# amcolex/ofdm-sync-math

Measured on AMD Instinct MI355X. Metric: complex Msamples/s through S&C metric kernel @ batch=65536; % HBM roofline, higher is better.
Workload: dtype f32 (c64 in, f64 prefix sums); 1 GPU; cfg3 Schmidl-Cox float32 metric+CFO, N=1024 (L=512), cir1, 65536 streams x 1024 c64 per GPU; global_batch=65536, seq_len=1024, L=512, parallelism=stream-shard x1 (no collectives), placement=auto -> contiguous

## Files before the change

### ofdm-sync-math_amd/csrc/aa_fast.hip

```cpp
#include "ofs_common.h"
#include "aa_gate.h"
#include "ofdmsync.h"

using namespace ofs;

namespace {

#ifndef OFS_FAST_WG
#define OFS_FAST_WG 64
#endif
constexpr int FAST_WG = OFS_FAST_WG;

#ifndef OFS_FAST_WAVES
#define OFS_FAST_WAVES 0
#endif
#if OFS_FAST_WAVES > 0
#define OFS_FAST_BOUNDS __launch_bounds__(FAST_WG, OFS_FAST_WAVES)
#else
#define OFS_FAST_BOUNDS __launch_bounds__(FAST_WG)
#endif
constexpr int TMAX = 1024;
constexpr int FAST_CAP_LDS = 160 * 1024 / 10;

#ifndef OFS_DMA_AUX
#define OFS_DMA_AUX 0
#endif
#ifndef OFS_FAST_STAGE
#define OFS_FAST_STAGE 1
#endif
typedef float nf4 __attribute__((ext_vector_type(4)));
typedef float nf2 __attribute__((ext_vector_type(2)));
typedef float pf2 __attribute__((ext_vector_type(2)));
__device__ __forceinline__ pf2 mulc_acc(pf2 c, pf2 d, pf2 acc) {
    acc = __builtin_elementwise_fma(c, d.xx, acc);
    return __builtin_elementwise_fma(c.yx, pf2{d.y, -d.y}, acc);
}
template <int SP>
__device__ __forceinline__ void st_out(float4* p, float4 v) {
    const nf4 d = nf4{v.x, v.y, v.z, v.w};
    if constexpr (SP == 1) __builtin_nontemporal_store(d, reinterpret_cast<nf4*>(p));
    else *p = v;
}
template <int SP>
__device__ __forceinline__ void st_out(float2* p, float2 v) {
    const nf2 d = nf2{v.x, v.y};
    if constexpr (SP == 1) __builtin_nontemporal_store(d, reinterpret_cast<nf2*>(p));
    else *p = v;
}

template <int SP>
__device__ __forceinline__ void st_rows2(float* span, const float (&a)[2], const float (&b)[2], int lane) {
    const bool odd = (lane & 1) != 0;
    const int idx = (lane < 32 ? 2 * lane : 2 * lane - 63) * 4;
    float o[4];
#pragma unroll
    for (int e = 0; e < 2; ++e) {
        const int ai = __float_as_int(a[e]), bi = __float_as_int(b[e]);
        const int bdn = dpp_i<0xA0>(bi);
        const int aup = dpp_i<0xF5>(ai);
        const int we = odd ? bdn : ai;
        const int wo = odd ? bi : aup;
        o[e] = __int_as_float(__builtin_amdgcn_ds_bpermute(idx, we));
        o[2 + e] = __int_as_float(__builtin_amdgcn_ds_bpermute(idx, wo));
    }
    st_out<SP>(reinterpret_cast<float4*>(span) + lane, make_float4(o[0], o[1], o[2], o[3]));
}


#ifndef OFS_FAST_FF
#define OFS_FAST_FF 0
#endif
#ifndef OFS_FAST_GATE_LATE
#define OFS_FAST_GATE_LATE 0
#endif
#ifndef OFS_FAST_HEADSCAN
#define OFS_FAST_HEADSCAN 0
#endif
template <int E, int MR, int NA, bool DO, bool S32, int SV = 0>
__global__ OFS_FAST_BOUNDS void aa_fast_kernel(AaFastArgs a) {
    static_assert(SV == 0 || (E == 2 && NA == 1 && !DO), "store-path variants: one-antenna E = 2 storing kernel");
    constexpr int SP = SV & 1;
    constexpr bool RP = (SV & 2) != 0;
    constexpr int RL = 64 * E;
    constexpr int RW = TMAX / RL;
    constexpr int L = MR * RL;
    constexpr int V4 = E / 2;
    static_assert(MR >= 1 && MR <= RW, "window must fit the stream tile");
#if OFS_FAST_STAGE == 0
    __shared__ float4 lds[FAST_WG / 64][NA * RW * V4][64];
#endif
    const int lane = threadIdx.x & 63;
    const int w = threadIdx.x >> 6;
    const int64_t b = (int64_t)(NA == 1 ? blockIdx.x : xcd_block()) * (FAST_WG / 64) + w;
    if (b >= a.B) return;
    const int T = (int)a.T;
#if OFS_FAST_STAGE == 0
    constexpr int SPR = V4 + ((E % 4 != 0) ? 2 * V4 : 2 * (V4 / 2));
#pragma unroll
    for (int k = 0; k < RW; ++k)
#pragma unroll
        for (int t = 0; t < NA; ++t) {
            const float2* xs = reinterpret_cast<const float2*>(a.x) + (b * NA + t) * a.T;
#pragma unroll
            for (int j = 0; j < V4; ++j) {
                int n = RL * k + E * lane + 2 * j;
                n = n < T ? n : T - 2;
                ofs::lds_dma16(xs + n, &lds[w][(t * RW + k) * V4 + j][0]);
            }
        }
    auto ldrow = [&](int t, int k, int j) { return lds[w][(t * RW + k) * V4 + j][lane]; };
    const bool all_out = !DO && !RP && a.P && a.R && a.M;
    auto row_wait = [&](int k) {
        if (all_out) ofs::vmcnt_wait((RW - 1 - k) * NA * V4 + k * SPR);
        else ofs::vmcnt_wait((RW - 1 - k) * NA * V4);
    };
#elif OFS_FAST_STAGE == 2
    constexpr int SPR = V4 + ((E % 4 != 0) ? 2 * V4 : 2 * (V4 / 2));
    nf4 xreg[NA][RW][V4];
#pragma unroll
    for (int k = 0; k < RW; ++k)
#pragma unroll
        for (int t = 0; t < NA; ++t) {
            const float2* xs = reinterpret_cast<const float2*>(a.x) + (b * NA + t) * a.T;
#pragma unroll
            for (int j = 0; j < V4; ++j) {
                int n = RL * k + E * lane + 2 * j;
                n = n < T ? n : T - 2;
                asm volatile("global_load_dwordx4 %0, %1, off" : "=v"(xreg[t][k][j]) : "v"(xs + n) : "memory");
            }
        }
    const bool count_st = !DO && !RP && a.P && a.R && a.M && T == TMAX;
    auto ldrow = [&](int t, int k, int j) { const nf4 v = xreg[t][k][j]; return make_float4(v.x, v.y, v.z, v.w); };
    auto row_wait = [&](int k) {
        if (count_st) ofs::vmcnt_wait((RW - 1 - k) * NA * V4 + k * SPR);
        else ofs::vmcnt_wait((RW - 1 - k) * NA * V4);
#pragma unroll
        for (int t = 0; t < NA; ++t)
#pragma unroll
            for (int j = 0; j < V4; ++j) asm volatile("" : "+v"(xreg[t][k][j]));
    };
#else
    float4 xreg[NA][RW][V4];
#pragma unroll
    for (int t = 0; t < NA; ++t) {
        const float2* xs = reinterpret_cast<const float2*>(a.x) + (b * NA + t) * a.T;
#pragma unroll
        for (int k = 0; k < RW; ++k)
#pragma unroll
            for (int j = 0; j < V4; ++j) {
                int n = RL * k + E * lane + 2 * j;
                n = n < T ? n : T - 2;
                xreg[t][k][j] = *reinterpret_cast<const float4*>(xs + n);
            }
    }
    auto ldrow = [&](int t, int k, int j) { return xreg[t][k][j]; };
    auto row_wait = [&](int) {};
#endif
    auto xrow = [&](int t, int k, pf2 (&c)[E]) {
#pragma unroll
        for (int j = 0; j < V4; ++j) {
            const bool ok = RL * k + E * lane + 2 * j < T;
            const float4 v = ldrow(t, k, j);
            c[2 * j] = ok ? pf2{v.x, v.y} : pf2{0.f, 0.f};
            c[2 * j + 1] = ok ? pf2{v.z, v.w} : pf2{0.f, 0.f};
        }
    };

    pf2 sS[MR][E];
    float sE[MR][E];
    double Cr[RW + 1], Ci[RW + 1], Ce[RW + 1];
    Cr[0] = Ci[0] = Ce[0] = 0.0;

    AaRowGate<E, float, false, (bool)(DO || OFS_FAST_FF || NA == 1)> gate;
#if OFS_FAST_GATE_LATE
    constexpr int GR = RW - MR > 0 ? RW - MR : 1;
    __shared__ float4 gl[FAST_WG / 64][GR][E][64];
#endif
    if (a.detect)
        gate.init(a.hyst, L, a.thr, a.fs, a.max_ev, a.ev_i + b * (int64_t)a.max_ev * 4,
                  a.ev_r + b * (int64_t)a.max_ev * 4);

    float* Pout = DO ? nullptr : reinterpret_cast<float*>(a.P);
    float* Rout = DO ? nullptr : reinterpret_cast<float*>(a.R);
    float* Mout = DO ? nullptr : reinterpret_cast<float*>(a.M);
    const float floor_ = 1e-6f * (float)L;
    float hR[2] = {0.f, 0.f}, hM[2] = {0.f, 0.f};
    const bool head = !DO && a.head_resident != 0;

#pragma unroll
    for (int k = 0; k < RW; ++k) {
        if (RL * k < T) {
            const int nb = RL * k + E * lane;
            pf2 av[E];
            float aE[E];
#pragma unroll
            for (int e = 0; e < E; ++e) { av[e] = pf2{0.f, 0.f}; aE[e] = 0.f; }
            row_wait(k);
#pragma unroll
            for (int t = 0; t < NA; ++t) {
                pf2 c[E];
                xrow(t, k, c);
#pragma unroll
                for (int e = 0; e < E; ++e) aE[e] += fmaf(c[e].x, c[e].x, c[e].y * c[e].y);
                if (k >= MR) {
                    pf2 d[E];
                    xrow(t, k - MR, d);
#pragma unroll
                    for (int e = 0; e < E; ++e) av[e] = mulc_acc(c[e], d[e], av[e]);
                }
            }
            pf2 fS[E], gS[E];
            float fE[E], gE[E];
            fS[0] = av[0]; fE[0] = aE[0];
#pragma unroll
            for (int e = 1; e < E; ++e) { fS[e] = fS[e - 1] + av[e]; fE[e] = fE[e - 1] + aE[e]; }
            gS[E - 1] = pf2{0.f, 0.f}; gE[E - 1] = 0.f;
#pragma unroll
            for (int e = E - 2; e >= 0; --e) { gS[e] = gS[e + 1] + av[e + 1]; gE[e] = gE[e + 1] + aE[e + 1]; }
            const RowScan sEr = row_scan<S32>(fE[E - 1]);
            RowScan sRr{0.f, 0.f, 0.0}, sIr{0.f, 0.f, 0.0};
            if (k >= MR || OFS_FAST_HEADSCAN) { sRr = row_scan<S32>(fS[E - 1].x); sIr = row_scan<S32>(fS[E - 1].y); }
            const double totR = sRr.tot, totI = sIr.tot, totE = sEr.tot;
            const pf2 xS = pf2{sRr.x, sIr.x};
            const float xE = sEr.x;
            const pf2 uS = pf2{sRr.u, sIr.u};
            const float uE = sEr.u;
            Cr[k + 1] = Cr[k] + totR; Ci[k + 1] = Ci[k] + totI; Ce[k + 1] = Ce[k] + totE;
            const pf2 wS = pf2{(float)((k >= MR) ? (Cr[k] - Cr[k - MR + 1]) : Cr[k]),
                               (float)((k >= MR) ? (Ci[k] - Ci[k - MR + 1]) : Ci[k])};
            const float wE = (float)((k >= MR) ? (Ce[k] - Ce[k - MR + 1]) : Ce[k]);

            float pf[E][2], mf[E], pmf[E], rf[E];
#pragma unroll
            for (int e = 0; e < E; ++e) {
                pf2 P = wS + (xS + fS[e]);
                float RR = wE + (xE + fE[e]);
                if (k >= MR) { P += sS[k % MR][e]; RR += sE[k % MR][e]; }
                sS[k % MR][e] = uS + gS[e]; sE[k % MR][e] = uE + gE[e];
                const float pm = fmaf(P.x, P.x, P.y * P.y);
                float m = 0.f;
                if (k >= MR && RR > floor_) m = fminf(pm * __builtin_amdgcn_rcpf(RR * RR), 1.f);
                pf[e][0] = P.x; pf[e][1] = P.y; rf[e] = RR; mf[e] = m; pmf[e] = pm;
            }

            const int64_t o = b * a.T + nb;
            float* const Pk = (k < MR && head) ? nullptr : Pout;
            float* const Mk = (k < MR && head) ? nullptr : Mout;
            const bool paired = RP && (T & 3) == 0 && RL * ((k & ~1) + 2) <= T;
#pragma unroll
            for (int j = 0; j < V4; ++j) {
                if (nb + 2 * j < T) {
                    if (Pk) st_out<SP>(reinterpret_cast<float4*>(Pk + 2 * (o + 2 * j)),
                                         make_float4(pf[2 * j][0], pf[2 * j][1], pf[2 * j + 1][0], pf[2 * j + 1][1]));
                    if (paired) {
                    } else if (E % 4 != 0 || (T & 3) != 0) {
                        if (Rout) st_out<SP>(reinterpret_cast<float2*>(Rout + o + 2 * j), make_float2(rf[2 * j], rf[2 * j + 1]));
                        if (Mk) st_out<SP>(reinterpret_cast<float2*>(Mk + o + 2 * j), make_float2(mf[2 * j], mf[2 * j + 1]));
                    } else if ((j & 1) == 0) {
                        if (Rout) st_out<SP>(reinterpret_cast<float4*>(Rout + o + 2 * j),
                                             make_float4(rf[2 * j], rf[2 * j + 1], rf[2 * j + 2], rf[2 * j + 3]));
                        if (Mk) st_out<SP>(reinterpret_cast<float4*>(Mk + o + 2 * j),
                                             make_float4(mf[2 * j], mf[2 * j + 1], mf[2 * j + 2], mf[2 * j + 3]));
                    }
                    if (!DO && a.valid) { a.valid[o + 2 * j] = (k >= MR); a.valid[o + 2 * j + 1] = (k >= MR); }
                }
            }
            if constexpr (RP) {
                if (paired) {
                    if ((k & 1) == 0) {
                        hR[0] = rf[0]; hR[1] = rf[1]; hM[0] = mf[0]; hM[1] = mf[1];
                    } else {
                        const int64_t o0 = b * a.T + RL * (k - 1);
                        if (Rout) st_rows2<SP>(Rout + o0, hR, rf, lane);
                        if (Mk) st_rows2<SP>(Mk + o0, hM, mf, lane);
                    }
                }
            }

            if (a.detect && k >= MR) {
#if OFS_FAST_GATE_LATE
#pragma unroll
                for (int e = 0; e < E; ++e) gl[w][k >= MR ? k - MR : 0][e][lane] = make_float4(mf[e], pmf[e], pf[e][0], pf[e][1]);
#else
                float pr[E], pi[E];
#pragma unroll
                for (int e = 0; e < E; ++e) { pr[e] = pf[e][0]; pi[e] = pf[e][1]; }
                gate.row(lane, k, nb, T, mf, pmf, pr, pi);
#endif
            }
        }
    }
#if OFS_FAST_GATE_LATE
    if (a.detect) {
        __builtin_amdgcn_fence(__ATOMIC_RELEASE, "wavefront");
        __builtin_amdgcn_wave_barrier();
        __builtin_amdgcn_fence(__ATOMIC_ACQUIRE, "wavefront");
#pragma unroll 1
        for (int k = MR; k < RW; ++k) {
            if (RL * k >= T) break;
            float m[E], pm[E], pr[E], pi[E];
#pragma unroll
            for (int e = 0; e < E; ++e) {
                const float4 v = gl[w][k - MR][e][lane];
                m[e] = v.x; pm[e] = v.y; pr[e] = v.z; pi[e] = v.w;
            }
            gate.row(lane, k, RL * k + E * lane, T, m, pm, pr, pi);
        }
    }
#endif
    if (a.detect) gate.finish(lane, T, a.n_ev + b);
}

typedef float f4u __attribute__((ext_vector_type(4), aligned(8)));
typedef float f2u __attribute__((ext_vector_type(2), aligned(4)));

#ifndef OFS_STREAM_WG
#define OFS_STREAM_WG 64
#endif
constexpr int STREAM_WG = OFS_STREAM_WG;
#ifndef OFS_STREAM_PD
#define OFS_STREAM_PD 0
#endif
#ifndef OFS_STREAM_WAVES
#define OFS_STREAM_WAVES 0
#endif
#ifndef OFS_STREAM_WG1
#define OFS_STREAM_WG1 128
#endif
constexpr int stream_wg(int na, bool det_only) { return (na == 1 && !det_only) ? OFS_STREAM_WG1 : STREAM_WG; }
#if OFS_STREAM_WAVES > 0
#define OFS_STREAM_BOUNDS __launch_bounds__(stream_wg(NA, DO), OFS_STREAM_WAVES)
#else
#define OFS_STREAM_BOUNDS __launch_bounds__(stream_wg(NA, DO))
#endif

#ifndef OFS_STREAM_FF
#define OFS_STREAM_FF 1
#endif
#ifndef OFS_STREAM_LDSLAG
#define OFS_STREAM_LDSLAG 1
#endif

template <int E, int MR, int NA, bool DO>
struct AaStream {
    static constexpr int RL = 64 * E;
    static constexpr int L = MR * RL;
    static constexpr int V4 = E / 2;
    static constexpr int PD = OFS_STREAM_PD > 0 ? OFS_STREAM_PD : ((E == 2 && NA == 2) ? 4 : 2);
    static constexpr int PER = MR > PD ? MR : PD;
    static constexpr bool LDSLAG = OFS_STREAM_LDSLAG == 2 || (OFS_STREAM_LDSLAG == 1 && NA == 2);

    const float2* xb;
    float4 (*lag)[NA][V4][64];
    int64_t T, o0;
    int Ti, nrows, full_rows, lane;
    pf2 lx[LDSLAG ? 1 : NA][MR][E];
    pf2 sS[MR][E];
    float sE[MR][E];
    double cbR[MR], cbI[MR], cbE[MR];
    double CR, CI, CE;
    float2 nx[PD][NA][E];
    AaRowGate<E, float, false, (bool)(DO || OFS_STREAM_FF)> gate;
    float2* Pout; float* Rout; float* Mout; uint8_t* Vout;
// ... 170 lines not shown
        if (p < s.nrows) s.load_row(p, s.nx[p]);
    s.detect = a.detect != 0;
    if (s.detect)
        s.gate.init(a.hyst, S::L, a.thr, a.fs, a.max_ev, a.ev_i + b * (int64_t)a.max_ev * 4,
                    a.ev_r + b * (int64_t)a.max_ev * 4);
    s.Pout = DO ? nullptr : reinterpret_cast<float2*>(a.P);
    s.Rout = DO ? nullptr : reinterpret_cast<float*>(a.R);
    s.Mout = DO ? nullptr : reinterpret_cast<float*>(a.M);
    s.Vout = DO ? nullptr : a.valid;
    s.head = !DO && a.head_resident != 0;
    s.floor_ = 1e-6f * (float)S::L;

    s.template block<true, true>(0);
    int k0 = S::PER;
    for (; k0 + S::PER + S::PD <= s.full_rows; k0 += S::PER) s.template block<false, false>(k0);
    for (; k0 < s.nrows; k0 += S::PER) s.template block<false, true>(k0);
    if (a.detect) s.gate.finish(lane, s.Ti, a.n_ev + b);
}

template <int E, int MR, int NA>
int launch_stream(const AaFastArgs& a, hipStream_t st) {
    const bool det_only = a.detect && !a.P && !a.R && !a.M && !a.valid;
    constexpr int WGD = stream_wg(NA, true), WGS = stream_wg(NA, false);
    const int64_t grid = det_only ? (a.B + WGD / 64 - 1) / (WGD / 64) : (a.B + WGS / 64 - 1) / (WGS / 64);
    using S = AaStream<E, MR, NA, false>;
    constexpr size_t lag_lds = (size_t)(WGS / 64) * (S::LDSLAG ? MR : 1) * NA * S::V4 * 64 * 16;
    constexpr size_t cap_total = 24 * 1024;
    const size_t dflt = (!det_only && NA == 2 && cap_total > lag_lds) ? cap_total - lag_lds : 0;
    const size_t shm = ofs::variant(ofs::V_OCC_LDS) == INT64_MIN ? dflt : ofs::occ_lds();
    if (det_only)
        hipLaunchKernelGGL((aa_stream_kernel<E, MR, NA, true>), dim3((unsigned)grid), dim3(WGD), shm, st, a);
    else
        hipLaunchKernelGGL((aa_stream_kernel<E, MR, NA, false>), dim3((unsigned)grid), dim3(WGS), shm, st, a);
    return hipGetLastError() == hipSuccess ? 1 : OFS_EHIP;
}

template <int E, int NA>
int launch_stream_mr(int mr, const AaFastArgs& a, hipStream_t st) {
    switch (mr) {
        case 1: return launch_stream<E, 1, NA>(a, st);
        case 2: return launch_stream<E, 2, NA>(a, st);
        case 4: return launch_stream<E, 4, NA>(a, st);
        case 8: return launch_stream<E, 8, NA>(a, st);
    }
    return 0;
}

bool scan32(bool det_only) {
    const int64_t v = ofs::variant(det_only ? ofs::V_FAST_SCAN_DO : ofs::V_FAST_SCAN);
    if (v == 32 || v == 64) return v == 32;
    return det_only;
}

template <int E, int MR, int NA>
int launch(const AaFastArgs& a, hipStream_t st) {
    const bool det_only = a.detect && !a.P && !a.R && !a.M && !a.valid;
    const bool s32 = scan32(det_only);
    const dim3 grid((unsigned)((a.B + FAST_WG / 64 - 1) / (FAST_WG / 64))), blk(FAST_WG);
    const int64_t pad = ofs::variant_or(ofs::V_FAST_LDS, (!det_only && NA == 1) ? FAST_CAP_LDS : 0);
    const size_t shm = pad > 0 && pad <= 65536 ? (size_t)pad : 0;
    if constexpr (E == 2 && NA == 1) {
        if (!det_only && !s32) {
            const int sv = (ofs::variant_or(ofs::V_FAST_RMPAIR, 1) != 0 ? 2 : 0) | (ofs::variant_or(ofs::V_FAST_ST_POLICY, 1) == 1 ? 1 : 0);
            switch (sv) {
                case 0: hipLaunchKernelGGL((aa_fast_kernel<E, MR, NA, false, false, 0>), grid, blk, shm, st, a); break;
                case 1: hipLaunchKernelGGL((aa_fast_kernel<E, MR, NA, false, false, 1>), grid, blk, shm, st, a); break;
                case 2: hipLaunchKernelGGL((aa_fast_kernel<E, MR, NA, false, false, 2>), grid, blk, shm, st, a); break;
                default: hipLaunchKernelGGL((aa_fast_kernel<E, MR, NA, false, false, 3>), grid, blk, shm, st, a);
            }
            return hipGetLastError() == hipSuccess ? 1 : OFS_EHIP;
        }
    }
    if (det_only && s32) hipLaunchKernelGGL((aa_fast_kernel<E, MR, NA, true, true>), grid, blk, shm, st, a);
    else if (det_only) hipLaunchKernelGGL((aa_fast_kernel<E, MR, NA, true, false>), grid, blk, shm, st, a);
    else if (s32) hipLaunchKernelGGL((aa_fast_kernel<E, MR, NA, false, true>), grid, blk, shm, st, a);
    else hipLaunchKernelGGL((aa_fast_kernel<E, MR, NA, false, false>), grid, blk, shm, st, a);
    return hipGetLastError() == hipSuccess ? 1 : OFS_EHIP;
}

template <int E, int NA, int MR = 1>
int launch_mr(int mr, const AaFastArgs& a, hipStream_t st) {
    if constexpr (MR > TMAX / (64 * E)) {
        return 0;
    } else {
        if (mr == MR) return launch<E, MR, NA>(a, st);
        return launch_mr<E, NA, MR + 1>(mr, a, st);
    }
}

template <int NA>
int launch_e(int E, int mr, const AaFastArgs& a, hipStream_t st) {
    switch (E) {
        case 2: return launch_mr<2, NA>(mr, a, st);
        case 4: return launch_mr<4, NA>(mr, a, st);
        case 8: return launch_mr<8, NA>(mr, a, st);
    }
    return 0;
}

int pick_e(int L) {
    const int forced = (int)ofs::variant_or(ofs::V_FAST_E, 0);
    if (forced == 2 || forced == 4 || forced == 8) return (L % (64 * forced) == 0) ? forced : 0;
    for (int e : {2, 4, 8})
        if (L % (64 * e) == 0) return e;
    return 0;
}

int pick_e_do(int L) {
    const int forced = (int)ofs::variant_or(ofs::V_FAST_E_DO, 0);
    for (int e : {forced, 4, 8, 2})
        if ((e == 2 || e == 4 || e == 8) && L % (64 * e) == 0) return e;
    return 0;
}

}

// ... 33 lines not shown
```

### ofdm-sync-math_amd/csrc/aa_gate.h

```cpp
#pragma once
#include "ofs_common.h"

namespace ofs {

#ifndef OFS_GATE_FASTFLAGS
#define OFS_GATE_FASTFLAGS 1
#endif
#ifndef OFS_GATE_PRED
#define OFS_GATE_PRED 0
#endif
#ifndef OFS_GATE_NOINLINE_EMIT
#define OFS_GATE_NOINLINE_EMIT 0
#endif
#ifndef OFS_GATE_FFONLY
#define OFS_GATE_FFONLY 0
#endif
#ifndef OFS_GATE_DIAG
#define OFS_GATE_DIAG 0
#endif
#ifndef OFS_GATE_NOACC
#define OFS_GATE_NOACC 0
#endif
#ifndef OFS_GATE_DEFER
#define OFS_GATE_DEFER 1
// ... 25 lines not shown
        lane_reset();
    }

#if OFS_GATE_NOINLINE_EMIT
    __device__ __attribute__((noinline)) void emit(int lane, int gate_end) {
#else
    __device__ __forceinline__ void emit(int lane, int gate_end) {
#endif
        if (evi && n_ev < max_ev && lane < 8) {
            int64_t* ei = evi + (int64_t)n_ev * 4;
            if constexpr (RTL) {
                const int64_t f[4] = {bidx, (int64_t)bidx + toff, ev_start, (int64_t)gate_end + 1};
                if (lane < 4) ei[lane] = f[lane & 3];
            } else {
                double* er = evr + (int64_t)n_ev * 4;
                const int64_t f[4] = {out_peak(), out_start(), out_pos(gate_end), out_peak() - 2 * L + 1};
                if (lane < 4) {
                    ei[lane] = f[lane & 3];
                } else {
                    const double ang = sizeof(V) == 4 ? (double)fast_atan2f((float)bpi, (float)bpr)
                                                      : atan2((double)bpi, (double)bpr);
                    const double g[4] = {(double)bpr, (double)bpi, (double)bm, ang * fs / (2.0 * M_PI * (double)L)};
                    er[lane - 4] = g[lane & 3];
                }
            }
        }
        n_ev += 1;
    }

    __device__ __forceinline__ void row(int lane, int k, int nb, int T, const V (&m)[E], const V (&pm)[E],
                                        const V (&pr)[E], const V (&pi)[E]) {
#if OFS_GATE_DIAG == 1
        return;
#endif
        bool ab[E];
#pragma unroll
        for (int e = 0; e < E; ++e) ab[e] = (nb + e < T) && (double)m[e] >= thr;
#if OFS_GATE_DIAG == 2
        uint64_t any = 0;
#pragma unroll
        for (int e = 0; e < E; ++e) any |= __ballot(ab[e]);
        if (any) carry_last = RL * k;
        return;
#endif
        row_flags(lane, k, nb, T, ab, pm, pr, pi, m);
    }

    V lv, lpr, lpi, lm;
    int lk;
    __device__ __forceinline__ void lane_reset() {
        lv = (V)-1; lpr = (V)0; lpi = (V)0; lm = (V)0;
        lk = RTL ? -1 : ABS_NOKEY;
    }
    __device__ __forceinline__ void accumulate(int lane, int k, int nb, int T, int lo, int hi, const V (&pm)[E],
                                               const V (&pr)[E], const V (&pi)[E], const V (&m)[E]) {
#if OFS_GATE_NOACC == 1
        return;
#endif
#pragma unroll
        for (int e = 0; e < E; ++e) {
            const int key = E * lane + e;
            const bool in = nb + e < T && key >= lo && key <= hi;
            const bool better = RTL ? (pm[e] >= lv) : (pm[e] > lv);
#if OFS_GATE_NOACC == 2
            if (in && better) { lv = pm[e]; lk = RL * k + key; }
#else
            if (in && better) { lv = pm[e]; lk = RL * k + key; lpr = pr[e]; lpi = pi[e]; lm = m[e]; }
#endif
        }
    }
#if OFS_GATE_NOINLINE_EMIT
    __device__ __attribute__((noinline)) void merge() {
#else
    __device__ __forceinline__ void merge() {
#endif
        const V vmax = wave_max(lv);
        const int kk = RTL ? wave_max_i(lv == vmax ? lk : -1) : wave_min(lv == vmax ? lk : ABS_NOKEY);
        const bool found = RTL ? (kk >= 0) : (kk != ABS_NOKEY);
        const bool take = RTL ? (vmax >= bpm) : (vmax > bpm);
        if (found && take) {
            const int ln = (kk % RL) / E;
            bpr = readlane(lpr, ln);
            bpi = readlane(lpi, ln);
            bm = readlane(lm, ln);
            bpm = vmax;
            bidx = kk;
        }
        lane_reset();
    }
    __device__ __forceinline__ void seg(int lane, int k, int nb, int T, int lo, int hi, const V (&pm)[E],
                                        const V (&pr)[E], const V (&pi)[E], const V (&m)[E]) {
        accumulate(lane, k, nb, T, lo, hi, pm, pr, pi, m);
        if (!(DEFER && OFS_GATE_DEFER)) merge();
    }
    __device__ __forceinline__ void open_at(int start) {
        gate_open = 1; ev_start = start; bpm = (V)-1; lane_reset();
    }

    __device__ __forceinline__ void row_flags(int lane, int k, int nb, int T, const bool (&ab)[E],
                                              const V (&pm)[E], const V (&pr)[E], const V (&pi)[E],
                                              const V (&m)[E]) {
#if OFS_GATE_PRED
        if (FF && DEFER && OFS_GATE_DEFER && Hp >= RL) {
            int first = GATE_NOKEY, last = -1;
#pragma unroll
            for (int e = 0; e < E; ++e) {
                const uint64_t am = __ballot(ab[e]);
                const int f = am ? E * (int)__builtin_ctzll(am) + e : GATE_NOKEY;
                const int l = am ? E * (63 - (int)__builtin_clzll(am)) + e : -1;
                first = min(first, f);
                last = max(last, l);
            }
            const int base = RL * k;
            const int c = carry_last + Hp;
            if (carry_last >= 0 && c >= base && c < base + RL && c < T && c - base < first) {
                accumulate(lane, k, nb, T, gate_open ? 0 : -1, c - base, pm, pr, pi, m);
                merge();
                emit(lane, c);
                gate_open = 0;
            }
            const bool has = first != GATE_NOKEY;
            const bool opens = has && (carry_last < 0 || base + first - 1 - carry_last >= Hp);
            carry_last = has ? base + last : carry_last;
            ev_start = opens ? base + first : ev_start;
            bpm = opens ? (V)-1 : bpm;
            lv = opens ? (V)-1 : lv;
            lk = opens ? (RTL ? -1 : ABS_NOKEY) : lk;
            const int lo = opens ? first : (gate_open ? 0 : RL);
            gate_open = (opens || gate_open) ? 1 : 0;
            accumulate(lane, k, nb, T, lo, RL - 1, pm, pr, pi, m);
            return;
        }
#endif
        if (FF && OFS_GATE_FASTFLAGS && (OFS_GATE_FFONLY || Hp >= RL)) {
            int first = GATE_NOKEY, last = -1;
#pragma unroll
            for (int e = 0; e < E; ++e) {
                const uint64_t am = __ballot(ab[e]);
                if (am) {
                    first = min(first, E * (int)__builtin_ctzll(am) + e);
                    last = max(last, E * (63 - (int)__builtin_clzll(am)) + e);
                }
            }
            const int base = RL * k;
            int seg_lo = gate_open ? 0 : -1;
            if (carry_last >= 0) {
                const int c = carry_last + Hp;
                if (c >= base && c < base + RL && c < T && c - base < first) {
                    seg(lane, k, nb, T, seg_lo, c - base, pm, pr, pi, m);
                    if (DEFER && OFS_GATE_DEFER) merge();
                    emit(lane, c);
                    gate_open = 0; seg_lo = -1;
                }
            }
            if (first != GATE_NOKEY) {
                const int f = base + first;
                if (carry_last < 0 || f - 1 - carry_last >= Hp) {
                    open_at(f); seg_lo = first;
                }
                carry_last = base + last;
            }
            if (gate_open) seg(lane, k, nb, T, seg_lo, RL - 1, pm, pr, pi, m);
            return;
        }
#if OFS_GATE_FFONLY
        return;
#endif
        int lane_last = -1;
#pragma unroll
        for (int e = 0; e < E; ++e)
            if (ab[e]) lane_last = nb + e;
        const int W = max(wave_scan_max(lane_last, lane), carry_last);
        int run = wave_shr1(W, lane, carry_last);
        uint64_t Om[E], Cm[E];
        uint64_t any = 0;
#pragma unroll
        for (int e = 0; e < E; ++e) {
            const int n = nb + e;
            const int pe = run;
            if (ab[e]) run = n;
            const bool cl = (n < T) && run >= 0 && (n - run) == Hp;
            const bool op = ab[e] && (pe < 0 || (n - 1 - pe) >= Hp);
            Om[e] = __ballot(op);
            Cm[e] = __ballot(cl);
            any |= Om[e] | Cm[e];
        }
        carry_last = readlane(W, 63);

        int seg_lo = gate_open ? 0 : -1;
        if (any) {
            int pos = -1;
            while (true) {
                int key = GATE_NOKEY, is_open = 0;
#pragma unroll
                for (int e = 0; e < E; ++e) {
                    const int q = pos - e;
                    const int t = q < 0 ? 0 : q / E + 1;
                    const uint64_t msk = t >= 64 ? 0ull : (~0ull << t);
                    const uint64_t o = Om[e] & msk, c = Cm[e] & msk;
                    if (o) { const int kq = E * __builtin_ctzll(o) + e; if (kq < key) { key = kq; is_open = 1; } }
                    if (c) { const int kq = E * __builtin_ctzll(c) + e; if (kq < key) { key = kq; is_open = 0; } }
                }
                if (key == GATE_NOKEY) break;
                if (is_open) {
                    open_at(RL * k + key); seg_lo = key;
                } else {
                    seg(lane, k, nb, T, seg_lo, key, pm, pr, pi, m);
                    if (DEFER && OFS_GATE_DEFER) merge();
                    emit(lane, RL * k + key);
                    gate_open = 0; seg_lo = -1;
                }
                pos = key;
            }
        }
        if (gate_open) seg(lane, k, nb, T, seg_lo, RL - 1, pm, pr, pi, m);
    }

    __device__ __forceinline__ void finish(int lane, int T, int32_t* n_ev_out, int64_t* open_start = nullptr) {
        if constexpr (RTL) {
            if (lane == 0) {
                *n_ev_out = n_ev;
                if (open_start) *open_start = gate_open ? ev_start : -1;
            }
        } else {
            if (gate_open) { if (DEFER && OFS_GATE_DEFER) merge(); emit(lane, T); }
            if (lane == 0) *n_ev_out = n_ev;
        }
    }

    __device__ __forceinline__ int64_t out_pos(int g) const {
        if constexpr (ABS) return (int64_t)g + this->abs0;
        else return g;
    }
    __device__ __forceinline__ int64_t out_peak() const {
        if constexpr (ABS) return bidx == CARRIED ? this->b0_abs : out_pos(bidx);
        else return bidx;
    }
    __device__ __forceinline__ int64_t out_start() const {
        if constexpr (ABS) return ev_start == CARRIED ? this->ev0_abs : out_pos(ev_start);
        else return ev_start;
    }


    __device__ __forceinline__ void load(int64_t abs0_, int64_t carry_p1, int open, int64_t ev_start_abs,
                                         int64_t bidx_abs, V bpm_, V bpr_, V bpi_, V bm_) {
        static_assert(ABS && !RTL, "resumable form of the sync_aa machine");
        this->abs0 = abs0_; this->ev0_abs = ev_start_abs; this->b0_abs = bidx_abs;
        const int64_t cg = carry_p1 - 1 - abs0_;
        carry_last = (carry_p1 > 0 && cg >= 0) ? (int)cg : -1;
        if (open) {
            gate_open = 1; ev_start = CARRIED; bidx = CARRIED;
            bpm = bpm_; bpr = bpr_; bpi = bpi_; bm = bm_;
        }
    }
    __device__ __forceinline__ void save(int64_t& carry_p1, int& open, int64_t& ev_start_abs, int64_t& bidx_abs) const {
        static_assert(ABS && !RTL, "resumable form of the sync_aa machine");
        carry_p1 = carry_last >= 0 ? out_pos(carry_last) + 1 : 0;
        open = gate_open;
        ev_start_abs = out_start();
        bidx_abs = out_peak();
    }
};

}
```

### ofdm-sync-math_amd/csrc/ofdmsync.hip

```cpp
#include <hip/hip_runtime.h>
#include <stdint.h>
#include <math.h>
#include "ofdmsync.h"
#include "ofs_common.h"
#include <atomic>
#include <string.h>

namespace {

constexpr int WG = 256;
constexpr int EPT = 4;
constexpr int ROW = 64 * EPT;
constexpr int PASS = WG * EPT;
constexpr int EVBLK = 1024;
constexpr int MAXSLOT = 32;

enum Mode { M_AA = 0, M_SC = 1, M_COMB = 2, M_MINN = 3, M_RTL = 4 };

template <bool EX> struct Prec { using R = float; };
template <> struct Prec<true> { using R = double; };

template <int FMT, class R>
__device__ __forceinline__ void ldx(const void* p, int64_t i, R& re, R& im) {
    if constexpr (FMT == OFS_C64) {
// ... 674 lines not shown
    if (p.lds > 65536) {
        if (hipFuncSetAttribute((const void*)k, hipFuncAttributeMaxDynamicSharedMemorySize, (int)p.lds) != hipSuccess)
            return OFS_EHIP;
    }
    a.chunk = p.chunk; a.n_chunks = p.n_chunks; a.len_max = p.len_max; a.nrows_max = p.nrows_max;
    const int64_t grid = B * (int64_t)p.n_chunks;
    if (grid > 0x7fffffffll) return OFS_EINVAL;
    hipLaunchKernelGGL(k, dim3((unsigned)grid), dim3(WG), p.lds, st, a);
    return hipGetLastError() == hipSuccess ? OFS_OK : OFS_EHIP;
}

template <int MODE>
static int dispatch_win(int fmt, int precision, WinArgs a, int64_t B, int lo_x, int hi_x,
                        hipStream_t st, Plan* plan_out) {
    constexpr int nq = NQ<MODE>::v;
    Plan p;
    int rc;
    const bool ex = precision == OFS_FP64;
    rc = ex ? make_plan<double>(a.T, a.n_out, lo_x, hi_x, nq, true, p)
            : make_plan<float>(a.T, a.n_out, lo_x, hi_x, nq, false, p);
    if (rc) return rc;
    if (plan_out) *plan_out = p;
    a.lo_x = lo_x; a.hi_x = hi_x;
    if (ex) {
        switch (fmt) {
            case OFS_C64: return launch_win<OFS_C64, true, MODE>(a, B, p, st);
            case OFS_C128: return launch_win<OFS_C128, true, MODE>(a, B, p, st);
            case OFS_CI16: return launch_win<OFS_CI16, true, MODE>(a, B, p, st);
        }
    } else if constexpr (MODE != M_RTL) {
        switch (fmt) {
            case OFS_C64: return launch_win<OFS_C64, false, MODE>(a, B, p, st);
            case OFS_C128: return launch_win<OFS_C128, false, MODE>(a, B, p, st);
            case OFS_CI16: return launch_win<OFS_CI16, false, MODE>(a, B, p, st);
        }
    }
    return OFS_EINVAL;
}

static bool fmt_ok(int f) { return f == OFS_C64 || f == OFS_C128 || f == OFS_CI16; }
static bool prec_ok(int p) { return p == OFS_FP32 || p == OFS_FP64; }

}

extern "C" {

int32_t ofs_version(void) { return 100; }


static const char* const kVariantNames[ofs::V_COUNT] = {
    "EXACT", "FAST_E", "FAST_E_DO", "FAST_SCAN", "FAST_SCAN_DO", "RTL_WPB", "PARK_DIRECT", "ZW64",
    "ZW64_GRID", "ZS", "ZF_ITEMS", "ZS_PAIR", "ZS_DEFER", "ZS_BPL", "ZS_C", "ZS_GBLK", "MC_FUSED",
    "MC_FUSE_X", "ZC_SEQ", "ZC_NODMA", "BE_FAST", "MC_PERS", "FAST_LDS", "OCC_LDS",
    "FAST_RMPAIR", "FAST_ST_POLICY", "FAST_HEAD"};
struct VariantTable {
    int64_t v[ofs::V_COUNT];
    VariantTable() { for (auto& x : v) x = OFS_VARIANT_UNSET; }
};
static thread_local VariantTable g_variants;

static int variant_index(const char* name) {
    if (!name) return -1;
    for (int i = 0; i < ofs::V_COUNT; ++i)
        if (strcmp(name, kVariantNames[i]) == 0) return i;
    return -1;
}

int32_t ofs_debug_reset_variants(void) {
    for (auto& x : g_variants.v) x = OFS_VARIANT_UNSET;
    return OFS_OK;
}

int32_t ofs_debug_set_variant(const char* name, int64_t value) {
    const int i = variant_index(name);
    if (i < 0) return OFS_EINVAL;
    g_variants.v[i] = value;
    return OFS_OK;
}

int64_t ofs_debug_get_variant(const char* name) {
    const int i = variant_index(name);
    return i < 0 ? OFS_VARIANT_UNSET : ofs::variant((ofs::Variant)i);
}

const char* ofs_status_string(int32_t s) {
    switch (s) {
        case OFS_OK: return "ok";
        case OFS_EINVAL: return "invalid argument";
        case OFS_ETOOLONG: return "window/halo does not fit one LDS tile";
        case OFS_EHIP: return "HIP launch error";
        case OFS_ESHORT: return "stream shorter than one symbol";
        case OFS_EFFT: return "rocFFT error";
        default: return "unknown status";
    }
}

int32_t ofs_aa_detect(int32_t in_fmt, const void* x, int64_t B, int32_t n_ant, int64_t T,
                      int32_t L, int32_t precision, void* P, void* R, void* M, uint8_t* valid,
                      int32_t detect, double threshold, int32_t hysteresis, double sample_rate,
                      int32_t max_events, int32_t* n_events, int64_t* ev_int, double* ev_real,
                      void* stream) {
    return ofs_aa_detect_ex(in_fmt, x, B, n_ant, T, L, precision, P, R, M, valid, detect, threshold, hysteresis,
                            sample_rate, max_events, n_events, ev_int, ev_real, stream, 0u);
}

int32_t ofs_aa_detect_ex(int32_t in_fmt, const void* x, int64_t B, int32_t n_ant, int64_t T,
                         int32_t L, int32_t precision, void* P, void* R, void* M, uint8_t* valid,
// ... 235 lines not shown
```

### ofdm-sync-math_amd/csrc/ofs_common.h

```cpp
#pragma once
#include <hip/hip_runtime.h>
#include <stdint.h>

#define OFS_MISSING(p, n) ((p) == nullptr && (int64_t)(n) > 0)

namespace ofs {

enum Variant : int {
    V_EXACT, V_FAST_E, V_FAST_E_DO, V_FAST_SCAN, V_FAST_SCAN_DO, V_RTL_WPB, V_PARK_DIRECT, V_ZW64,
    V_ZW64_GRID, V_ZS, V_ZF_ITEMS, V_ZS_PAIR, V_ZS_DEFER, V_ZS_BPL, V_ZS_C, V_ZS_GBLK, V_MC_FUSED,
    V_MC_FUSE_X, V_ZC_SEQ, V_ZC_NODMA, V_BE_FAST, V_MC_PERS, V_FAST_LDS, V_OCC_LDS,
    V_FAST_RMPAIR, V_FAST_ST_POLICY, V_FAST_HEAD, V_COUNT
};
int64_t variant(Variant v);
inline bool variant_is(Variant v, int64_t value) { return variant(v) == value; }
inline bool variant_off(Variant v) { return variant(v) == 0; }
inline bool variant_on(Variant v) { const int64_t x = variant(v); return x != INT64_MIN && x != 0; }
inline int64_t variant_or(Variant v, int64_t dflt) { const int64_t x = variant(v); return x == INT64_MIN ? dflt : x; }
inline size_t occ_lds() { const int64_t x = variant(V_OCC_LDS); return x > 0 && x <= 65536 ? (size_t)x : 0; }


template <int CTRL>
__device__ __forceinline__ int dpp_i(int v) {
    return __builtin_amdgcn_mov_dpp(v, CTRL, 0xf, 0xf, false);
}
template <int CTRL>
__device__ __forceinline__ double dpp_d(double v) {
    const int lo = dpp_i<CTRL>(__double2loint(v));
    const int hi = dpp_i<CTRL>(__double2hiint(v));
    return __hiloint2double(hi, lo);
}

__device__ __forceinline__ double wave_scan_add(double v, int lane) {
    const int rl = lane & 15;
    double t;
    t = dpp_d<0x111>(v); if (rl >= 1) v += t;
    t = dpp_d<0x112>(v); if (rl >= 2) v += t;
    t = dpp_d<0x114>(v); if (rl >= 4) v += t;
    t = dpp_d<0x118>(v); if (rl >= 8) v += t;
    t = dpp_d<0x142>(v); if ((lane & 31) >= 16) v += t;
    t = dpp_d<0x143>(v); if (lane >= 32) v += t;
    return v;
}

__device__ __forceinline__ int wave_scan_max(int v, int lane) {
    const int rl = lane & 15;
    int t;
    t = dpp_i<0x111>(v); if (rl >= 1) v = max(v, t);
    t = dpp_i<0x112>(v); if (rl >= 2) v = max(v, t);
    t = dpp_i<0x114>(v); if (rl >= 4) v = max(v, t);
    t = dpp_i<0x118>(v); if (rl >= 8) v = max(v, t);
    t = dpp_i<0x142>(v); if ((lane & 31) >= 16) v = max(v, t);
    t = dpp_i<0x143>(v); if (lane >= 32) v = max(v, t);
    return v;
}

__device__ __forceinline__ double wave_shr1(double v, int lane, double first) {
    const double t = dpp_d<0x138>(v);
    return lane == 0 ? first : t;
}
__device__ __forceinline__ int wave_shr1(int v, int lane, int first) {
    const int t = dpp_i<0x138>(v);
    return lane == 0 ? first : t;
}

// ... 124 lines not shown
    v += dppz_f<0x118>(v);
    v += dppz_f<0x142, 0xa>(v);
    v += dppz_f<0x143, 0xc>(v);
    return v;
}

struct RowScan { float x, u; double tot; };
template <bool F32>
__device__ __forceinline__ RowScan row_scan(float v) {
    if constexpr (F32) {
        const float i = scan_add_f32(v);
        const float t = readlane(i, 63);
        return RowScan{dppz_f<0x138>(i), t - i, (double)t};
    } else {
        const double i = scan_add((double)v);
        const double t = readlane(i, 63);
        return RowScan{(float)shr1z(i), (float)(t - i), t};
    }
}


__device__ __forceinline__ void lds_dma16(const void* g, const void* lds) {
    const uint32_t m = (uint32_t)(uintptr_t)(__attribute__((address_space(3))) const void*)lds;
    asm volatile("s_mov_b32 m0, %1\n\ts_nop 0\n\tglobal_load_lds_dwordx4 %0, off" ::"v"(g), "s"(m) : "memory", "m0");
}


#define OFS_VMW(i) case i: asm volatile("s_waitcnt vmcnt(" #i ")" ::: "memory"); break;
__device__ __forceinline__ void vmcnt_wait(int n) {
    switch (n < 63 ? n : 63) {
        OFS_VMW(0) OFS_VMW(1) OFS_VMW(2) OFS_VMW(3) OFS_VMW(4) OFS_VMW(5) OFS_VMW(6) OFS_VMW(7)
        OFS_VMW(8) OFS_VMW(9) OFS_VMW(10) OFS_VMW(11) OFS_VMW(12) OFS_VMW(13) OFS_VMW(14) OFS_VMW(15)
        OFS_VMW(16) OFS_VMW(17) OFS_VMW(18) OFS_VMW(19) OFS_VMW(20) OFS_VMW(21) OFS_VMW(22) OFS_VMW(23)
        OFS_VMW(24) OFS_VMW(25) OFS_VMW(26) OFS_VMW(27) OFS_VMW(28) OFS_VMW(29) OFS_VMW(30) OFS_VMW(31)
        OFS_VMW(32) OFS_VMW(33) OFS_VMW(34) OFS_VMW(35) OFS_VMW(36) OFS_VMW(37) OFS_VMW(38) OFS_VMW(39)
        OFS_VMW(40) OFS_VMW(41) OFS_VMW(42) OFS_VMW(43) OFS_VMW(44) OFS_VMW(45) OFS_VMW(46) OFS_VMW(47)
        OFS_VMW(48) OFS_VMW(49) OFS_VMW(50) OFS_VMW(51) OFS_VMW(52) OFS_VMW(53) OFS_VMW(54) OFS_VMW(55)
        OFS_VMW(56) OFS_VMW(57) OFS_VMW(58) OFS_VMW(59) OFS_VMW(60) OFS_VMW(61) OFS_VMW(62)
        default: asm volatile("s_waitcnt vmcnt(63)" ::: "memory"); break;
    }
}
#undef OFS_VMW

}

struct AaFastArgs {
    const void* x;
    int64_t B, T;
    int32_t L;
    void* P; void* R; void* M; uint8_t* valid;
    int32_t detect; double thr; int32_t hyst; double fs;
    int32_t max_ev; int32_t* n_ev; int64_t* ev_i; double* ev_r;
    int32_t head_resident;
};
int ofs_aa_fast_try(int fmt, int precision, int n_ant, const AaFastArgs& a, hipStream_t st);
int ofs_aa_fast_plan(int fmt, int precision, int n_ant, int64_t T, int L);

int ofs_aa_exact_plan(int fmt, int precision, int n_ant, int64_t T, int L);
int ofs_aa_exact_try(int fmt, int precision, int n_ant, const AaFastArgs& a, hipStream_t st);
struct RtlExactCall {
    const void* x; int64_t B, T; int32_t Q;
    int32_t shift, smooth_mode, frac_bits; double thr_value;
    double* corr_total; double* corr_positive; double* smooth; double* energy_total;
    double* corr_scaled; double* energy_scaled; uint8_t* mvalid; uint8_t* above;
    int32_t detect, hyst, toff, max_ev; int32_t* n_ev; int64_t* ev; int64_t* open_start;
};
int ofs_rtl_exact_plan(int fmt, int n_br, int64_t T, int Q);
int ofs_rtl_exact_try(int fmt, int n_br, const RtlExactCall& c, hipStream_t st);

struct WinFastArgs {
    const void* x; int64_t B, T; int N;
    void* M; void* P; void* R;
};
int ofs_win_fast_try(int mode, int fmt, int precision, int n_br, const WinFastArgs& a, hipStream_t st);
int ofs_win_fast_plan(int mode, int fmt, int precision, int n_br, int64_t T, int N);
int ofs_sc_minn_fast_plan(int fmt, int precision, int n_br, int64_t T, int N);
int ofs_sc_minn_fast_try(int fmt, int precision, int n_br, const void* x, int64_t B, int64_t T, int N,
                         void* Ms, void* Ps, void* Rs, void* Mm, void* Pm, void* Rm, hipStream_t st);
```

Baseline: 332,400 Msamples/s.

## Add full-stream specialized fast kernel with compile-time bounds and fast-flag gate

Adds a template specialization (FS) of the fast Schmidl-Cox kernel for the case T==1024 with all outputs and detection enabled. It removes per-element tail bounds checks, uses byte-offset addressing with precomputed lane offsets, and writes P/R/M through a simplified store path. The detection gate is forced into the fast-flags mode (or the ballot path when hysteresis is small), using a precomputed float32 threshold instead of comparing in the generic path. It also sets a different default LDS padding to tune occupancy. The specialization adds code complexity and relies on the threshold rounding matching the double comparison.

```diff
diff --git a/ofdm-sync-math_amd/csrc/aa_fast.hip b/ofdm-sync-math_amd/csrc/aa_fast.hip
--- a/ofdm-sync-math_amd/csrc/aa_fast.hip
+++ b/ofdm-sync-math_amd/csrc/aa_fast.hip
@@ -1,3 +1,5 @@
+#include <cfloat>
+#include <cmath>
 #include "ofs_common.h"
 #include "aa_gate.h"
 #include "ofdmsync.h"
@@ -21,6 +23,7 @@
 #endif
 constexpr int TMAX = 1024;
 constexpr int FAST_CAP_LDS = 160 * 1024 / 10;
+constexpr int FAST_CAP_LDS_FULL = 23000;
 
 #ifndef OFS_DMA_AUX
 #define OFS_DMA_AUX 0
@@ -76,9 +79,11 @@
 #ifndef OFS_FAST_HEADSCAN
 #define OFS_FAST_HEADSCAN 0
 #endif
-template <int E, int MR, int NA, bool DO, bool S32, int SV = 0>
+template <int E, int MR, int NA, bool DO, bool S32, int SV = 0, int FS = 0>
 __global__ OFS_FAST_BOUNDS void aa_fast_kernel(AaFastArgs a) {
     static_assert(SV == 0 || (E == 2 && NA == 1 && !DO), "store-path variants: one-antenna E = 2 storing kernel");
+    static_assert(FS == 0 || (SV == 3 && !S32 && OFS_FAST_STAGE == 1 && !OFS_FAST_GATE_LATE), "full-stream form: the headline's kernel");
+    constexpr bool FULL = FS != 0;
     constexpr int SP = SV & 1;
     constexpr bool RP = (SV & 2) != 0;
     constexpr int RL = 64 * E;
@@ -90,10 +95,11 @@
     __shared__ float4 lds[FAST_WG / 64][NA * RW * V4][64];
 #endif
     const int lane = threadIdx.x & 63;
-    const int w = threadIdx.x >> 6;
+    const int w = (FULL && FAST_WG == 64) ? 0 : threadIdx.x >> 6;
     const int64_t b = (int64_t)(NA == 1 ? blockIdx.x : xcd_block()) * (FAST_WG / 64) + w;
     if (b >= a.B) return;
-    const int T = (int)a.T;
+    const int T = FULL ? TMAX : (int)a.T;
+    const uint32_t lo16 = 16u * (uint32_t)lane;
 #if OFS_FAST_STAGE == 0
     constexpr int SPR = V4 + ((E % 4 != 0) ? 2 * V4 : 2 * (V4 / 2));
 #pragma unroll
@@ -141,6 +147,11 @@
     };
 #else
     float4 xreg[NA][RW][V4];
+    if constexpr (FULL) {
+        const char* const xb = reinterpret_cast<const char*>(a.x) + b * (TMAX * 8);
+#pragma unroll
+        for (int k = 0; k < RW; ++k) xreg[0][k][0] = *reinterpret_cast<const float4*>(xb + RL * 8 * k + lo16);
+    } else {
 #pragma unroll
     for (int t = 0; t < NA; ++t) {
         const float2* xs = reinterpret_cast<const float2*>(a.x) + (b * NA + t) * a.T;
@@ -153,13 +164,14 @@
                 xreg[t][k][j] = *reinterpret_cast<const float4*>(xs + n);
             }
     }
+    }
     auto ldrow = [&](int t, int k, int j) { return xreg[t][k][j]; };
     auto row_wait = [&](int) {};
 #endif
     auto xrow = [&](int t, int k, pf2 (&c)[E]) {
 #pragma unroll
         for (int j = 0; j < V4; ++j) {
-            const bool ok = RL * k + E * lane + 2 * j < T;
+            const bool ok = FULL || RL * k + E * lane + 2 * j < T;
             const float4 v = ldrow(t, k, j);
             c[2 * j] = ok ? pf2{v.x, v.y} : pf2{0.f, 0.f};
             c[2 * j + 1] = ok ? pf2{v.z, v.w} : pf2{0.f, 0.f};
@@ -176,7 +188,8 @@
     constexpr int GR = RW - MR > 0 ? RW - MR : 1;
     __shared__ float4 gl[FAST_WG / 64][GR][E][64];
 #endif
-    if (a.detect)
+    const bool detect = FULL || a.detect;
+    if (detect)
         gate.init(a.hyst, L, a.thr, a.fs, a.max_ev, a.ev_i + b * (int64_t)a.max_ev * 4,
                   a.ev_r + b * (int64_t)a.max_ev * 4);
 
@@ -186,10 +199,13 @@
     const float floor_ = 1e-6f * (float)L;
     float hR[2] = {0.f, 0.f}, hM[2] = {0.f, 0.f};
     const bool head = !DO && a.head_resident != 0;
+    char* const Pb = FULL ? reinterpret_cast<char*>(a.P) + b * (TMAX * 8) : nullptr;
+    float* const Rb = FULL ? reinterpret_cast<float*>(a.R) + b * TMAX : nullptr;
+    float* const Mb = FULL ? reinterpret_cast<float*>(a.M) + b * TMAX : nullptr;
 
 #pragma unroll
     for (int k = 0; k < RW; ++k) {
-        if (RL * k < T) {
+        if (FULL || RL * k < T) {
             const int nb = RL * k + E * lane;
             pf2 av[E];
             float aE[E];
@@ -243,6 +259,16 @@
                 pf[e][0] = P.x; pf[e][1] = P.y; rf[e] = RR; mf[e] = m; pmf[e] = pm;
             }
 
+            if constexpr (FULL) {
+                const bool pm_row = !(k < MR && head);
+                if (pm_row) st_out<SP>(reinterpret_cast<float4*>(Pb + RL * 8 * k + lo16), make_float4(pf[0][0], pf[0][1], pf[1][0], pf[1][1]));
+                if ((k & 1) == 0) {
+                    hR[0] = rf[0]; hR[1] = rf[1]; hM[0] = mf[0]; hM[1] = mf[1];
+                } else {
+                    st_rows2<SP>(Rb + RL * (k - 1), hR, rf, lane);
+                    if (pm_row) st_rows2<SP>(Mb + RL * (k - 1), hM, mf, lane);
+                }
+            } else {
             const int64_t o = b * a.T + nb;
             float* const Pk = (k < MR && head) ? nullptr : Pout;
             float* const Mk = (k < MR && head) ? nullptr : Mout;
@@ -276,8 +302,9 @@
                     }
                 }
             }
-
-            if (a.detect && k >= MR) {
+            }
+
+            if (detect && k >= MR) {
 #if OFS_FAST_GATE_LATE
 #pragma unroll
                 for (int e = 0; e < E; ++e) gl[w][k >= MR ? k - MR : 0][e][lane] = make_float4(mf[e], pmf[e], pf[e][0], pf[e][1]);
@@ -285,7 +312,14 @@
                 float pr[E], pi[E];
 #pragma unroll
                 for (int e = 0; e < E; ++e) { pr[e] = pf[e][0]; pi[e] = pf[e][1]; }
-                gate.row(lane, k, nb, T, mf, pmf, pr, pi);
+                if constexpr (FULL) {
+                    bool ab[E];
+#pragma unroll
+                    for (int e = 0; e < E; ++e) ab[e] = mf[e] >= a.thr32;
+                    gate.template row_flags<FS, true>(lane, k, nb, T, ab, pmf, pr, pi, mf);
+                } else {
+                    gate.row(lane, k, nb, T, mf, pmf, pr, pi);
+                }
 #endif
             }
         }
@@ -308,7 +342,7 @@
         }
     }
 #endif
-    if (a.detect) gate.finish(lane, T, a.n_ev + b);
+    if (detect) gate.finish(lane, T, a.n_ev + b);
 }
 
 typedef float f4u __attribute__((ext_vector_type(4), aligned(8)));
@@ -585,6 +619,15 @@
     return det_only;
 }
 
+float thr_as_f32(double thr) {
+    if (thr != thr || thr == (double)INFINITY || thr == -(double)INFINITY) return (float)thr;
+    if (thr > (double)FLT_MAX) return INFINITY;
+    if (thr < -(double)FLT_MAX) return -FLT_MAX;
+    float f = (float)thr;
+    if ((double)f < thr) f = nextafterf(f, INFINITY);
+    return f;
+}
+
 template <int E, int MR, int NA>
 int launch(const AaFastArgs& a, hipStream_t st) {
     const bool det_only = a.detect && !a.P && !a.R && !a.M && !a.valid;
@@ -595,6 +638,20 @@
     if constexpr (E == 2 && NA == 1) {
         if (!det_only && !s32) {
             const int sv = (ofs::variant_or(ofs::V_FAST_RMPAIR, 1) != 0 ? 2 : 0) | (ofs::variant_or(ofs::V_FAST_ST_POLICY, 1) == 1 ? 1 : 0);
+            if constexpr (MR == 1 || MR == 2 || MR == 4) {
+                if (sv == 3 && a.T == TMAX && a.P && a.R && a.M && !a.valid && a.detect && a.n_ev && a.ev_i && a.ev_r &&
+                    !ofs::variant_off(ofs::V_FAST_FULL)) {
+                    AaFastArgs f = a;
+                    f.thr32 = thr_as_f32(a.thr);
+                    const int64_t padf = ofs::variant_or(ofs::V_FAST_LDS, FAST_CAP_LDS_FULL);
+                    const size_t shmf = padf > 0 && padf <= 65536 ? (size_t)padf : 0;
+                    if ((a.hyst > 1 ? a.hyst : 1) >= 64 * E)
+                        hipLaunchKernelGGL((aa_fast_kernel<E, MR, NA, false, false, 3, 1>), grid, blk, shmf, st, f);
+                    else
+                        hipLaunchKernelGGL((aa_fast_kernel<E, MR, NA, false, false, 3, 2>), grid, blk, shmf, st, f);
+                    return hipGetLastError() == hipSuccess ? 1 : OFS_EHIP;
+                }
+            }
             switch (sv) {
                 case 0: hipLaunchKernelGGL((aa_fast_kernel<E, MR, NA, false, false, 0>), grid, blk, shm, st, a); break;
                 case 1: hipLaunchKernelGGL((aa_fast_kernel<E, MR, NA, false, false, 1>), grid, blk, shm, st, a); break;
diff --git a/ofdm-sync-math_amd/csrc/aa_gate.h b/ofdm-sync-math_amd/csrc/aa_gate.h
--- a/ofdm-sync-math_amd/csrc/aa_gate.h
+++ b/ofdm-sync-math_amd/csrc/aa_gate.h
@@ -101,6 +101,7 @@
         lv = (V)-1; lpr = (V)0; lpi = (V)0; lm = (V)0;
         lk = RTL ? -1 : ABS_NOKEY;
     }
+    template <bool FULLROW = false>
     __device__ __forceinline__ void accumulate(int lane, int k, int nb, int T, int lo, int hi, const V (&pm)[E],
                                                const V (&pr)[E], const V (&pi)[E], const V (&m)[E]) {
 #if OFS_GATE_NOACC == 1
@@ -109,7 +110,7 @@
 #pragma unroll
         for (int e = 0; e < E; ++e) {
             const int key = E * lane + e;
-            const bool in = nb + e < T && key >= lo && key <= hi;
+            const bool in = (FULLROW || nb + e < T) && key >= lo && key <= hi;
             const bool better = RTL ? (pm[e] >= lv) : (pm[e] > lv);
 #if OFS_GATE_NOACC == 2
             if (in && better) { lv = pm[e]; lk = RL * k + key; }
@@ -137,15 +138,17 @@
         }
         lane_reset();
     }
+    template <bool FULLROW = false>
     __device__ __forceinline__ void seg(int lane, int k, int nb, int T, int lo, int hi, const V (&pm)[E],
                                         const V (&pr)[E], const V (&pi)[E], const V (&m)[E]) {
-        accumulate(lane, k, nb, T, lo, hi, pm, pr, pi, m);
+        accumulate<FULLROW>(lane, k, nb, T, lo, hi, pm, pr, pi, m);
         if (!(DEFER && OFS_GATE_DEFER)) merge();
     }
     __device__ __forceinline__ void open_at(int start) {
         gate_open = 1; ev_start = start; bpm = (V)-1; lane_reset();
     }
 
+    template <int MODE = 0, bool FULLROW = false>
     __device__ __forceinline__ void row_flags(int lane, int k, int nb, int T, const bool (&ab)[E],
                                               const V (&pm)[E], const V (&pr)[E], const V (&pi)[E],
                                               const V (&m)[E]) {
@@ -181,7 +184,7 @@
             return;
         }
 #endif
-        if (FF && OFS_GATE_FASTFLAGS && (OFS_GATE_FFONLY || Hp >= RL)) {
+        if (MODE == 1 || (MODE == 0 && FF && OFS_GATE_FASTFLAGS && (OFS_GATE_FFONLY || Hp >= RL))) {
             int first = GATE_NOKEY, last = -1;
 #pragma unroll
             for (int e = 0; e < E; ++e) {
@@ -195,8 +198,8 @@
             int seg_lo = gate_open ? 0 : -1;
             if (carry_last >= 0) {
                 const int c = carry_last + Hp;
-                if (c >= base && c < base + RL && c < T && c - base < first) {
-                    seg(lane, k, nb, T, seg_lo, c - base, pm, pr, pi, m);
+                if (c >= base && c < base + RL && (FULLROW || c < T) && c - base < first) {
+                    seg<FULLROW>(lane, k, nb, T, seg_lo, c - base, pm, pr, pi, m);
                     if (DEFER && OFS_GATE_DEFER) merge();
                     emit(lane, c);
                     gate_open = 0; seg_lo = -1;
@@ -209,7 +212,7 @@
                 }
                 carry_last = base + last;
             }
-            if (gate_open) seg(lane, k, nb, T, seg_lo, RL - 1, pm, pr, pi, m);
+            if (gate_open) seg<FULLROW>(lane, k, nb, T, seg_lo, RL - 1, pm, pr, pi, m);
             return;
         }
 #if OFS_GATE_FFONLY
@@ -228,7 +231,7 @@
             const int n = nb + e;
             const int pe = run;
             if (ab[e]) run = n;
-            const bool cl = (n < T) && run >= 0 && (n - run) == Hp;
+            const bool cl = (FULLROW || n < T) && run >= 0 && (n - run) == Hp;
             const bool op = ab[e] && (pe < 0 || (n - 1 - pe) >= Hp);
             Om[e] = __ballot(op);
             Cm[e] = __ballot(cl);
@@ -254,7 +257,7 @@
                 if (is_open) {
                     open_at(RL * k + key); seg_lo = key;
                 } else {
-                    seg(lane, k, nb, T, seg_lo, key, pm, pr, pi, m);
+                    seg<FULLROW>(lane, k, nb, T, seg_lo, key, pm, pr, pi, m);
                     if (DEFER && OFS_GATE_DEFER) merge();
                     emit(lane, RL * k + key);
                     gate_open = 0; seg_lo = -1;
@@ -262,7 +265,7 @@
                 pos = key;
             }
         }
-        if (gate_open) seg(lane, k, nb, T, seg_lo, RL - 1, pm, pr, pi, m);
+        if (gate_open) seg<FULLROW>(lane, k, nb, T, seg_lo, RL - 1, pm, pr, pi, m);
     }
 
     __device__ __forceinline__ void finish(int lane, int T, int32_t* n_ev_out, int64_t* open_start = nullptr) {
diff --git a/ofdm-sync-math_amd/csrc/ofdmsync.hip b/ofdm-sync-math_amd/csrc/ofdmsync.hip
--- a/ofdm-sync-math_amd/csrc/ofdmsync.hip
+++ b/ofdm-sync-math_amd/csrc/ofdmsync.hip
@@ -750,7 +750,7 @@
     "EXACT", "FAST_E", "FAST_E_DO", "FAST_SCAN", "FAST_SCAN_DO", "RTL_WPB", "PARK_DIRECT", "ZW64",
     "ZW64_GRID", "ZS", "ZF_ITEMS", "ZS_PAIR", "ZS_DEFER", "ZS_BPL", "ZS_C", "ZS_GBLK", "MC_FUSED",
     "MC_FUSE_X", "ZC_SEQ", "ZC_NODMA", "BE_FAST", "MC_PERS", "FAST_LDS", "OCC_LDS",
-    "FAST_RMPAIR", "FAST_ST_POLICY", "FAST_HEAD"};
+    "FAST_RMPAIR", "FAST_ST_POLICY", "FAST_HEAD", "FAST_FULL"};
 struct VariantTable {
     int64_t v[ofs::V_COUNT];
     VariantTable() { for (auto& x : v) x = OFS_VARIANT_UNSET; }
diff --git a/ofdm-sync-math_amd/csrc/ofs_common.h b/ofdm-sync-math_amd/csrc/ofs_common.h
--- a/ofdm-sync-math_amd/csrc/ofs_common.h
+++ b/ofdm-sync-math_amd/csrc/ofs_common.h
@@ -10,7 +10,7 @@
     V_EXACT, V_FAST_E, V_FAST_E_DO, V_FAST_SCAN, V_FAST_SCAN_DO, V_RTL_WPB, V_PARK_DIRECT, V_ZW64,
     V_ZW64_GRID, V_ZS, V_ZF_ITEMS, V_ZS_PAIR, V_ZS_DEFER, V_ZS_BPL, V_ZS_C, V_ZS_GBLK, V_MC_FUSED,
     V_MC_FUSE_X, V_ZC_SEQ, V_ZC_NODMA, V_BE_FAST, V_MC_PERS, V_FAST_LDS, V_OCC_LDS,
-    V_FAST_RMPAIR, V_FAST_ST_POLICY, V_FAST_HEAD, V_COUNT
+    V_FAST_RMPAIR, V_FAST_ST_POLICY, V_FAST_HEAD, V_FAST_FULL, V_COUNT
 };
 int64_t variant(Variant v);
 inline bool variant_is(Variant v, int64_t value) { return variant(v) == value; }
@@ -241,6 +241,7 @@
     int32_t detect; double thr; int32_t hyst; double fs;
     int32_t max_ev; int32_t* n_ev; int64_t* ev_i; double* ev_r;
     int32_t head_resident;
+    float thr32;
 };
 int ofs_aa_fast_try(int fmt, int precision, int n_ant, const AaFastArgs& a, hipStream_t st);
 int ofs_aa_fast_plan(int fmt, int precision, int n_ant, int64_t T, int L);
```

After: 343,700 Msamples/s (median of 6 runs). 1.03x the previous value.
